# talha-alam/ADAM-Dehaze

Measured on AMD Instinct MI355X. Metric: images/sec CORUN-Complex fwd+bwd 512x1024 bs=8; PSNR vs CPU ref, higher is better.
Workload: dtype f32; 1 GPU; CORUN-Complex (HighIntensityDehazeModel base 96) train-mode fwd + L1 + bwd + Adam; per_gpu_batch=8, global_batch=8, height=512, width=1024, parallelism=dp1

## Files before the change

adam-dehaze_amd/_hip.py:

```python
from __future__ import annotations

import ctypes as C
import os
from typing import Optional

import torch

_LIB_PATH = os.environ.get("ADH_LIB_PATH") or os.path.join(os.path.dirname(os.path.abspath(__file__)), "lib",
                                                           "libadamdehaze_hip.so")
_lib: Optional[C.CDLL] = None

ACT_NONE, ACT_RELU = 0, 1
ACT_RELU6, ACT_HARDSWISH, ACT_HARDSIGMOID = 4, 5, 6

i32, i64, f32, f64, vp = C.c_int32, C.c_int64, C.c_float, C.c_double, C.c_void_p


class ConvDesc(C.Structure):
    _fields_ = [
        ("in_", vp), ("out", vp), ("wp", vp), ("scale", vp), ("shift", vp), ("residual", vp), ("stats", vp),
        ("N", i32), ("IH", i32), ("IW", i32), ("Cin", i32), ("in_cstride", i32),
        ("OH", i32), ("OW", i32), ("Cout", i32), ("out_cstride", i32), ("res_cstride", i32),
        ("VH", i32), ("VW", i32),
        ("in_sy", i32), ("in_sx", i32),
# ... 31 lines not shown
        ("K", i32), ("Nc", i32), ("KHt", i32), ("KWt", i32),
        ("tap_off0", i32), ("tap_off_sy", i32), ("tap_off_sx", i32),
        ("stride_k", i32), ("stride_n", i32),
    ]


PD = C.POINTER(ConvDesc)
PL = C.POINTER(WLayout)

_SIGNATURES = {
    "adh_version": [],
    "adh_conv_lds_bytes": [PD],
    "adh_conv_num_blocks": [PD],
    "adh_pack_weights": [vp, vp, PL, vp],
    "adh_conv_forward": [vp, PD],
    "adh_conv_wino_supported": [PD],
    "adh_conv_wino_forward": [vp, PD],
    "adh_conv_wino_num_blocks": [PD],
    "adh_conv_wino32_supported": [PD],
    "adh_conv_wino32_num_blocks": [PD],
    "adh_conv_wino32_forward": [vp, PD],
    "adh_conv_wino32_forward_multi": [vp, PD, i32],
    "adh_pack_weights_wino32": [vp, vp, PL, vp],
    "adh_conv_wino32_forward_bf16x3": [vp, PD],
    "adh_conv_wino32_forward_multi_bf16x3": [vp, PD, i32],
    "adh_pack_weights_wino32_bf16x3": [vp, vp, PL, vp],
    "adh_conv_wino43_supported": [PD],
    "adh_conv_wino43_num_blocks": [PD],
    "adh_conv_wino43_forward": [vp, PD],
    "adh_conv_wino43_dgrad_bnred": [vp, PD, vp],
    "adh_pack_weights_wino43": [vp, vp, PL, vp],
    "adh_conv_wino43_set_persistent": [i32],
    "adh_conv_wino43_forward_bf16x3": [vp, PD],
    "adh_conv_wino43_dgrad_bnred_bf16x3": [vp, PD, vp],
    "adh_pack_weights_wino43_bf16x3": [vp, vp, PL, vp],
    "adh_pack_weights_wino": [vp, vp, PL, vp],
    "adh_conv_wgrad": [vp, PD, vp, i32],
    "adh_conv_wgrad_wino_groups": [PD],
    "adh_conv_wgrad_wino": [vp, PD, vp, i32],
    "adh_wgrad_reduce_wino": [vp, vp, i32, i32, i32, PL, vp, i32],
    "adh_conv_wgrad_wino32_groups": [PD],
    "adh_conv_wgrad_wino32_classes": [PD],
    "adh_conv_wgrad_wino32_tiles": [PD],
    "adh_conv_wgrad_wino32_launches": [PD],
    "adh_conv_wgrad_wino32": [vp, PD, vp, i32],
    "adh_conv_wgrad_wino32_multi": [vp, PD, i32, vp, i32],
# ... 120 lines not shown
    "adh_bn_slice_stats_num_blocks": [i64, i32],
    "adh_bn_slice_stats": [vp, vp, i32, i64, i32, vp],
    "adh_bn_slice_moments": [vp, vp, i32, i32, i32, f64, vp, vp],
    "adh_bn_fold_moments": [vp, i32, vp, vp, f64, vp, vp, f32, f32, vp, vp, vp, vp, vp, vp, vp],
    "adh_avgpool2_bwd": [vp, vp, i32, i32, i32, i32, i32, vp, i32, i32],
    "adh_bn_preact_bwd_accum": [vp, vp, i32, vp, i32, vp, vp, vp, vp, i32, vp, i32, i64, i32, i32],
    "adh_u8_to_image": [vp, vp, i64, i64, i32, i32, i32, i32, vp],
    "adh_image_to_u8": [vp, vp, i32, i32, i32, vp, i64, i64, i32],
    "adh_ciede2000_num_blocks": [i64],
    "adh_ciede2000": [vp, vp, vp, i32, i32, i32, i32, vp, i32, vp, vp],
    "adh_d4_apply": [vp, vp, i32, i32, i32, i32, i32, i32, vp, vp, i32, f32],
    "adh_msssim_num_tiles": [i32, i32],
    "adh_msssim_level_fwd": [vp, vp, vp, i32, i32, i32, i32, f64, vp, i32, vp, vp, vp, vp],
    "adh_msssim_level_bwd": [vp, vp, vp, i32, i32, i32, i32, f64, vp, vp, vp, vp, i32],
    "adh_draw_boxes": [vp, vp, i64, i64, i32, i32, i32, i32, vp, i32, vp, vp, vp, i32, vp, i32, i32, i32, i32],
    "adh_u8_resize_bilinear": [vp, vp, i64, i32, i32, i32, vp, i32, i32],
    "adh_batch_num_blocks": [i64],
    "adh_batch_from_u8": [vp, vp, i64, i64, i32, i32, vp, vp, i32, vp, i32, vp],
    "adh_batch_window_from_u8": [vp, vp, i64, vp, vp, i32, i32, i32, vp, i32, vp],
    "adh_nss_halve": [vp, vp, i32, i32, i32, i32, i32, i32, vp],
    "adh_nss_moments": [vp, vp, i32, i32, i32, i32, i32, i32, i32, i32, vp, i32, vp],
}

_VALUE_FUNCS = {"adh_version", "adh_conv_fewout_supported", "adh_conv_fewin_supported", "adh_conv_fewin_num_blocks", "adh_conv_wgrad_wino32_launches", "adh_conv_wino_supported", "adh_conv_wino_num_blocks", "adh_conv_wino32_supported", "adh_conv_wino43_supported", "adh_conv_wino43_num_blocks", "adh_conv_wino43_set_persistent",
                "adh_conv_wino32_num_blocks", "adh_conv_wgrad_wino_groups", "adh_conv_wgrad_wino32_groups", "adh_conv_wgrad_wino32_classes", "adh_conv_wgrad_wino32_tiles", "adh_conv_wgrad_wino43_groups", "adh_conv_wgrad_wino43_strips", "adh_conv_wgrad_small_slabs", "adh_conv_wgrad_stem_slabs", "adh_conv_stem_num_blocks", "adh_conv_wgrad_slabs", "adh_conv_wgrad_groups", "adh_conv_lds_bytes", "adh_conv_num_blocks", "adh_bn_bwd_num_blocks",
                "adh_cbam_pool_num_blocks", "adh_cbam_bwd_b_num_blocks", "adh_head_blend_bwd_num_blocks",
                "adh_reduce_num_blocks", "adh_lpips_layer_num_blocks", "adh_adam_chunk_elems", "adh_nms_words", "adh_augment_num_blocks", "adh_psnr_num_blocks", "adh_cbam_bwd_d_scratch_floats",
                "adh_ssim_num_blocks", "adh_fft_l1_workspace_bytes", "adh_fft_l1_num_partials", "adh_dwconv_num_blocks", "adh_dwconv_wgrad_num_blocks", "adh_channel_scale_bwd_num_blocks",
                "adh_bn_slice_stats_num_blocks", "adh_ciede2000_num_blocks", "adh_msssim_num_tiles", "adh_batch_num_blocks"}

_ERRORS = {-1: "ADH_E_ARG (bad argument: shape / alignment / null pointer)",
           -2: "ADH_E_LAUNCH (hip kernel launch failed)",
           -3: "ADH_E_UNSUPPORTED (configuration not supported by the kernels)"}


def lib_path() -> str:
    return _LIB_PATH


def load() -> C.CDLL:
    global _lib
    if _lib is None:
        if not os.path.exists(_LIB_PATH):
            raise RuntimeError(
                f"{_LIB_PATH} not found: the HIP extension is not built (run `python -c 'import __graft_entry__ as g; "
                "g.build()'` or `make -C adam-dehaze_amd/csrc`). There is no CPU fallback on the product path.")
        lib = C.CDLL(_LIB_PATH)
# ... 72 lines not shown
```

adam-dehaze_amd/csrc/conv_wino.hip:

```cpp
#include "common.h"
#ifndef W_STORE_AUX
#define W_STORE_AUX 0
#endif
#ifndef W3_DBG
#define W3_DBG 0
#endif
#include <cstdlib>
#include <cstring>
#define B3_NO_SPLIT ((W3_DBG & 16) != 0)
#include "bf16x3.h"

#define W2_KC 16
#define W2_TILES 64
#define W2_VBUF_F (16 * W2_TILES * W2_KC)
#define W2_RAW_PITCH 576
#define W2_RAW_F (10 * W2_RAW_PITCH)
#define W2_LDS_BYTES ((2 * W2_VBUF_F + W2_RAW_F) * 4)

typedef __attribute__((address_space(3))) void* lds_void_ptr;

struct WinoGeom {
    int tiles_x, tiles_y;
    int nregions;
    int nchunks;
    int KQtot;
    int ncog;
    int dbg;
};

template <int NT, int FT, int J>
constexpr bool w2_in_agpr() {
    constexpr int nv = 8 * NT - 16;
    if constexpr (nv <= 0) return true;
    else return !(J == 0 && FT >= 8 - nv);
}
template <bool AGPR>
__device__ __forceinline__ void w2_mfma(f32x16& c, float a, float b) {
    if constexpr (AGPR) asm("v_mfma_f32_32x32x2_f32 %0, %1, %2, %0" : "+a"(c) : "v"(a), "v"(b));
    else asm("v_mfma_f32_32x32x2_f32 %0, %1, %2, %0" : "+v"(c) : "v"(a), "v"(b));
}
template <int NT, int J, int FT, int R>
__device__ __forceinline__ void w2_store_m(const f32x16 (&acc)[8 * NT], unsigned addr) {
    if constexpr (FT < 8) {
        constexpr int off = ((FT >> 1) * W2_TILES + 8 * (R >> 2) + ((R & 3) << 1) + 32 * (FT & 1)) * 128;
        if constexpr (w2_in_agpr<NT, FT, J>())
            asm volatile("ds_write_b32 %0, %1 offset:%2" ::"v"(addr), "a"(acc[FT * NT + J][R]), "n"(off) : "memory");
        else
            asm volatile("ds_write_b32 %0, %1 offset:%2" ::"v"(addr), "v"(acc[FT * NT + J][R]), "n"(off) : "memory");
        if constexpr (R + 1 < 16) w2_store_m<NT, J, FT, R + 1>(acc, addr);
        else w2_store_m<NT, J, FT + 1, 0>(acc, addr);
    }
}

template <int NT, int F, int KK, int TH, int J, int KEND = 4>
__device__ __forceinline__ void w2_group(f32x16 (&acc)[8 * NT], const f32x4 (&a)[2], const f32x4 (&b)[NT]) {
    if constexpr (KK < KEND) {
        w2_mfma<w2_in_agpr<NT, F * 2 + TH, J>()>(acc[(F * 2 + TH) * NT + J], a[TH][KK], b[J][KK]);
        if constexpr (J + 1 < NT) w2_group<NT, F, KK, TH, J + 1, KEND>(acc, a, b);
        else if constexpr (TH == 0) w2_group<NT, F, KK, 1, 0, KEND>(acc, a, b);
        else w2_group<NT, F, KK + 1, 0, 0, KEND>(acc, a, b);
    }
}

template <int NT>
__device__ __forceinline__ void w2_load_b(f32x4 (&b)[NT], unsigned voff, const float* sbase) {
    asm volatile("global_load_dwordx4 %0, %1, %2" : "=v"(b[0]) : "v"(voff), "s"(sbase) : "memory");
    if constexpr (NT > 1) asm volatile("global_load_dwordx4 %0, %1, %2 offset:512" : "=v"(b[1]) : "v"(voff), "s"(sbase) : "memory");
    if constexpr (NT > 2) asm volatile("global_load_dwordx4 %0, %1, %2 offset:1024" : "=v"(b[2]) : "v"(voff), "s"(sbase) : "memory");
}
template <int N, int NT>
__device__ __forceinline__ void w2_wait_b(f32x4 (&b)[NT]) {
    if constexpr (NT == 1) asm volatile("s_waitcnt vmcnt(%1)" : "+v"(b[0]) : "n"(N) : "memory");
    if constexpr (NT == 2) asm volatile("s_waitcnt vmcnt(%2)" : "+v"(b[0]), "+v"(b[1]) : "n"(N) : "memory");
    if constexpr (NT == 3) asm volatile("s_waitcnt vmcnt(%3)" : "+v"(b[0]), "+v"(b[1]), "+v"(b[2]) : "n"(N) : "memory");
}

template <int NT>
__global__ __launch_bounds__(256, 1) void conv_wino_kernel(const adh_conv_desc d, const WinoGeom g) {
    extern __shared__ __attribute__((aligned(16))) float lds[];
    float* const raw = lds + 2 * W2_VBUF_F;

    const int tid = threadIdx.x;
    const int lane = tid & 63;
// ... 496 lines not shown
            }
            asm volatile("s_nop 1" : "+v"(a[0][0]), "+v"(a[0][1]), "+v"(a[0][2]), "+v"(a[1][0]), "+v"(a[1][1]), "+v"(a[1][2]));
        } else {
            w3b_gap<NT, FI, 12 * J + 12>(n, v0, v1, m1);
        }
        w3b_groups<NT, G + 1>(acc, a, n, bv, v0, v1, b_voff, b_slab, m1, st, sgn, nbuf);
    }
}

struct Wino32Geom {
    int tiles_x, tiles_y;
    int nregions;
    int nchunks;
    int KQtot;
    int ncog;
    int ncls, xps;
    int ymin[4], xmin[4];
    int wcls;
    int nmerge, mblocks;
    int region0;
    int m_out_oy[4], m_out_ox[4];
    const float* m_wp[4];
    float* m_stats[4];
};

template <int NT, bool BF3 = false>
__global__ __launch_bounds__(256, 1) void conv_wino32_kernel(const adh_conv_desc d, const Wino32Geom g) {
    extern __shared__ __attribute__((aligned(16))) float lds[];
    float* const rawbase = lds + W2_VBUF_F;
    float* const red = rawbase + 2 * W3_RAW_F;

    const int tid = threadIdx.x;
    const int lane = tid & 63;
    const int wave = __builtin_amdgcn_readfirstlane(tid >> 6);
    const int l31 = lane & 31;
    const int h = lane >> 5;

    const int bid = (int)blockIdx.x;
    const int gq = bid >> 3, per_region = g.ncog * g.nmerge;
    const int r8 = gq / per_region, rem = gq - r8 * per_region;
    const int mc = rem / g.ncog;
    const float* const wp_m = g.nmerge > 1 ? g.m_wp[mc] : d.wp;
    float* const stats_m = g.nmerge > 1 ? g.m_stats[mc] : d.stats;
    const int out_oy_m = g.nmerge > 1 ? g.m_out_oy[mc] : d.out_oy, out_ox_m = g.nmerge > 1 ? g.m_out_ox[mc] : d.out_ox;
    W3_STAMP(0);
#ifdef W3_PROF
    if (tid == 0 && bid < 16384) {
        w3_prof_buf[bid * 32 + 6] = __builtin_amdgcn_s_getreg((4 << 0) | (0 << 6) | (31 << 11));
        w3_prof_buf[bid * 32 + 7] = __builtin_amdgcn_s_getreg((20 << 0) | (0 << 6) | (31 << 11));
    }
#endif
    const int cg = rem - mc * g.ncog;
    const int region = g.region0 + r8 * 8 + (bid & 7);
    if (region >= g.nregions) return;
    int rr = region;
    const int tx = rr % g.tiles_x;
    rr /= g.tiles_x;
    const int ty = rr % g.tiles_y;
    const int n = rr / g.tiles_y;
    const int vy0 = ty * 12, vx0 = tx * 48;
    const int co0 = cg * 32 * NT;

    const int xcs = d.in_cstride * 4 * g.xps;
    const int xrs = d.IW * d.in_cstride * 4 * g.xps;
    const float* const in_n = d.in + (int64_t)n * d.IH * d.IW * d.in_cstride;
    const __amdgpu_buffer_rsrc_t xr = __builtin_amdgcn_make_buffer_rsrc(const_cast<float*>(in_n), 0, 0x7fffffff, 0x00020000);
    const int cq_l = lane & 3, px_l = lane >> 2;
    const int vfull = 3 * px_l * xcs + cq_l * 16;
    const int vtail = (px_l < W3_RAW_ROWS ? px_l : 0) * xrs + 48 * xcs + cq_l * 16;
    typedef W3Slab SlabGeom;
    auto slab_geom = [&](int slab) {
        SlabGeom sg;
        const int chunk = slab / g.ncls, c = slab - chunk * g.ncls;
        sg.iy0 = vy0 * g.xps + g.ymin[c + mc];
        sg.ix0 = vx0 * g.xps + g.xmin[c + mc];
        sg.interior = sg.iy0 >= 0 && sg.iy0 + 12 * g.xps < d.IH && sg.ix0 >= 0 && sg.ix0 + 48 * g.xps < d.IW;
// ... 15 lines not shown
                    __builtin_amdgcn_raw_ptr_buffer_load_lds(xr, (lds_void_ptr)(raw + r * W3_RAW_PITCH + p * 256), 16, vfull,
                                                             __builtin_amdgcn_readfirstlane(so0 + r * xrs + p * xcs), 0, 0);
                } else {
                    __builtin_amdgcn_raw_ptr_buffer_load_lds(xr, (lds_void_ptr)(raw + W3_RAW_ROWS * W3_RAW_PITCH), 16, vtail,
                                                             __builtin_amdgcn_readfirstlane(so0), 0, 0);
                }
            }
        } else {
#pragma unroll
            for (int u = u0; u < u1; ++u) {
                const int j = 4 * u + wv;
                const bool tail = j >= 39;
                const int rs = (j * 171) >> 9, p = tail ? 0 : j - rs * 3;
                const int r = tail ? (px_l < W3_RAW_ROWS ? px_l : 0) : rs;
                const int col = tail ? 48 : 3 * px_l + p;
                const int iy = iy0 + r * g.xps, ix = ix0 + col * g.xps;
                const bool ok = iy >= 0 && iy < d.IH && ix >= 0 && ix < d.IW;
                const int vo = ok ? (iy * d.IW + ix) * d.in_cstride * 4 + cq_l * 16 : (int)0x80000000;
                const int doff = __builtin_amdgcn_readfirstlane(tail ? W3_RAW_ROWS * W3_RAW_PITCH : rs * W3_RAW_PITCH + p * 256);
                __builtin_amdgcn_raw_ptr_buffer_load_lds(xr, (lds_void_ptr)(raw + doff), 16, vo, __builtin_amdgcn_readfirstlane(cb), 0, 0);
            }
        }
    };
    const int tcol = lane >> 2;
    const int tile_t = wave * 16 + tcol;
    int colb[3], colb3[4];
#pragma unroll
    for (int b = 0; b < 3; ++b) colb[b] = (3 * wave) * W3_RAW_PITCH + b * 256 + tcol * 16 + cq_l * 4;
#pragma unroll
    for (int i = 0; i < 4; ++i)
        colb3[i] = (tcol < 15 ? (3 * wave + i) * W3_RAW_PITCH + (tcol + 1) * 16 : W3_RAW_ROWS * W3_RAW_PITCH + (3 * wave + i) * 16) + cq_l * 4;
    const int vslot_t = tile_t * 16 + ((cq_l ^ ((tile_t >> 1) & 3)) * 4);
    const float m1 = adh_opaque(-1.f);
    auto transform = [&](int buf) {
        const float* raw = rawbase + buf * W3_RAW_F;
        float* Vb = lds + vslot_t;
#pragma unroll
        for (int a = 0; a < 4; ++a) {
            const int rA = a == 0 ? 0 : (a == 2 ? 2 : 1), rB = a == 0 ? 2 : (a == 1 ? 2 : (a == 2 ? 1 : 3));
            f32x4 t[4];
#pragma unroll
            for (int b = 0; b < 4; ++b) {
                const f32x4 dA = *reinterpret_cast<const f32x4*>(b < 3 ? raw + colb[b] + rA * W3_RAW_PITCH : raw + colb3[rA]);
                const f32x4 dB = *reinterpret_cast<const f32x4*>(b < 3 ? raw + colb[b] + rB * W3_RAW_PITCH : raw + colb3[rB]);
                t[b] = a == 1 ? dA + dB : adh_pksub(dA, dB, m1);
            }
            *reinterpret_cast<f32x4*>(Vb + (a * 4 + 0) * 1024) = adh_pksub(t[0], t[2], m1);
            *reinterpret_cast<f32x4*>(Vb + (a * 4 + 1) * 1024) = t[1] + t[2];
            *reinterpret_cast<f32x4*>(Vb + (a * 4 + 2) * 1024) = adh_pksub(t[2], t[1], m1);
            *reinterpret_cast<f32x4*>(Vb + (a * 4 + 3) * 1024) = adh_pksub(t[1], t[3], m1);
        }
    };

    const int sw = (l31 >> 1) & 3;
// ... 6 lines not shown
    f32x16 acc[8 * NT];
#pragma unroll
    for (int t = 0; t < 8 * NT; ++t)
#pragma unroll
        for (int r = 0; r < 16; ++r) acc[t][r] = 0.f;

    const float* const v0 = lds + a_lane;
    const float* const v1 = lds + (a_lane ^ 8);
    const unsigned b3_voff = (unsigned)lane * 16u;
    const size_t b3_chunk = (size_t)16 * NT * 3072, b3_cls = (size_t)g.ncog * g.nchunks * b3_chunk;
    const char* const b3_wave = reinterpret_cast<const char*>(wp_m) + ((size_t)cg * g.nchunks * 16 + (size_t)wave * 4) * (NT * 3072);
    auto b3_ptr = [&](int slab) {
        const int chunk = slab / g.ncls, c = slab - chunk * g.ncls;
        return b3_wave + (size_t)c * b3_cls + (size_t)chunk * b3_chunk;
    };
    W3Stage st3;
    st3.xr = xr; st3.rawbase = rawbase; st3.vfull = vfull; st3.vtail = vtail; st3.wave = wave; st3.px_l = px_l; st3.cq_l = cq_l;
    st3.xps = g.xps; st3.IH = d.IH; st3.IW = d.IW; st3.in_cstride = d.in_cstride; st3.xcs = xcs; st3.xrs = xrs;
    u32x4 av3[2][3], bv3[3][3];
    W4BNext nx[2];
    const float m1s = adh_opaque(-1.f);

    f32x4 av[2][2], bv[2][NT];
    auto load_a = [&](int f, int gg, f32x4 (&a)[2]) {
        const float* p = lds + f * 1024 + (gg ? (a_lane ^ 8) : a_lane);
        a[0] = *reinterpret_cast<const f32x4*>(p);
        a[1] = *reinterpret_cast<const f32x4*>(p + 512);
    };
    auto b_ptr = [&](int slab, int f, int gg) {
        const int chunk = slab / g.ncls, c = slab - chunk * g.ncls;
        return b_wave + (int64_t)c * g.wcls + f * b_fstride + (int64_t)(chunk * 4 + 2 * gg) * b_kqstride;
    };

    const int nslabs = g.nchunks * g.ncls;
    if constexpr (!BF3) w2_load_b<NT>(bv[0], b_voff, b_ptr(0, 0, 0));
    stage_raw(slab_geom(0), 0, 0, 10);
    asm volatile("s_waitcnt vmcnt(0)" ::: "memory");
    __builtin_amdgcn_s_barrier();
    if (!(W3_DBG & 1)) transform(0);
    asm volatile("s_waitcnt lgkmcnt(0)" ::: "memory");
    __builtin_amdgcn_s_barrier();

    W3_STAMP(1);
#pragma unroll 1
    for (int s = 0; s < nslabs; ++s) {
        if (s == 1) W3_STAMP(8);
        const int sn = s + 1 < nslabs ? s + 1 : s;
        constexpr int P = (W3_DBG & 8) ? 0 : 2;
        const SlabGeom sgn = slab_geom(sn);
        if constexpr (BF3) {
            if (!(W3_DBG & 2)) {
                w4b_load_b(bv3[0], b3_voff, b3_ptr(s));
                w4b_load_b(bv3[1], b3_voff, b3_ptr(s) + 3072);
                w3b_load_s(nx, v0, v1);
                w3b_steps<0, 40>(nx, m1s);
#pragma unroll
                for (int th = 0; th < 2; ++th) {
                    av3[th][0] = u32x4{nx[th].h[0], nx[th].h[1], nx[th].h[2], nx[th].h[3]};
                    av3[th][1] = u32x4{nx[th].m[0], nx[th].m[1], nx[th].m[2], nx[th].m[3]};
                    av3[th][2] = u32x4{nx[th].l[0], nx[th].l[1], nx[th].l[2], nx[th].l[3]};
                }
                asm volatile("s_nop 1" : "+v"(av3[0][0]), "+v"(av3[0][1]), "+v"(av3[0][2]), "+v"(av3[1][0]), "+v"(av3[1][1]), "+v"(av3[1][2]));
                w3b_load_s(nx, v0 + 1024, v1 + 1024);
                __builtin_amdgcn_sched_barrier(0);
                w3b_groups<NT, 0>(acc, av3, nx, bv3, v0, v1, b3_voff, b3_ptr(s), m1s, st3, sgn, (s + 1) & 1);
                asm volatile("s_waitcnt vmcnt(0)" ::: "memory");
            }
        } else if (!(W3_DBG & 2)) {
        load_a(0, 0, av[0]);
        w2_load_b<NT>(bv[1], b_voff, b_ptr(s, 1, 0));
        load_a(1, 0, av[1]);
        w2_wait_b<NT, NT>(bv[0]);
        w2_group<NT, 0, 0, 0, 0>(acc, av[0], bv[0]);

#define W3_GROUP_WITH_PIECES(F_, CUR, U0)                                             \
        w2_group<NT, F_, 0, 0, 0, 1>(acc, av[CUR], bv[CUR]);                           \
        __builtin_amdgcn_sched_barrier(0);                                            \
        if (P) stage_raw(sgn, (s + 1) & 1, U0, U0 + 2);                               \
        __builtin_amdgcn_sched_barrier(0);                                            \
        w2_group<NT, F_, 1, 0, 0>(acc, av[CUR], bv[CUR]);

        w2_load_b<NT>(bv[0], b_voff, b_ptr(s, 2, 0));
        load_a(2, 0, av[0]);
        w2_wait_b<NT, NT>(bv[1]);
        W3_GROUP_WITH_PIECES(1, 1, 0)

        w2_load_b<NT>(bv[1], b_voff, b_ptr(s, 3, 0));
        load_a(3, 0, av[1]);
        w2_wait_b<NT + P, NT>(bv[0]);
        W3_GROUP_WITH_PIECES(2, 0, 2)

        w2_load_b<NT>(bv[0], b_voff, b_ptr(s, 0, 1));
        load_a(0, 1, av[0]);
        w2_wait_b<NT + P, NT>(bv[1]);
        W3_GROUP_WITH_PIECES(3, 1, 4)

        w2_load_b<NT>(bv[1], b_voff, b_ptr(s, 1, 1));
        load_a(1, 1, av[1]);
        w2_wait_b<NT + P, NT>(bv[0]);
        W3_GROUP_WITH_PIECES(0, 0, 6)

        w2_load_b<NT>(bv[0], b_voff, b_ptr(s, 2, 1));
        load_a(2, 1, av[0]);
        w2_wait_b<NT + P, NT>(bv[1]);
        W3_GROUP_WITH_PIECES(1, 1, 8)
#undef W3_GROUP_WITH_PIECES

        w2_load_b<NT>(bv[1], b_voff, b_ptr(s, 3, 1));
        load_a(3, 1, av[1]);
        w2_wait_b<NT + P, NT>(bv[0]);
        w2_group<NT, 2, 0, 0, 0>(acc, av[0], bv[0]);

        w2_load_b<NT>(bv[0], b_voff, b_ptr(sn, 0, 0));
        w2_wait_b<NT, NT>(bv[1]);
        w2_group<NT, 3, 0, 0, 0>(acc, av[1], bv[1]);
        }
        if (s == 1) W3_STAMP(9);
        asm volatile("s_waitcnt lgkmcnt(0)" ::: "memory");
        __builtin_amdgcn_s_barrier();
        if (s == 1) W3_STAMP(10);
        if (!(W3_DBG & 1)) transform((s + 1) & 1);
        asm volatile("s_waitcnt lgkmcnt(0)" ::: "memory");
        if (s == 1) W3_STAMP(11);
        __builtin_amdgcn_s_barrier();
        if (s == 1) W3_STAMP(12);
    }
    if constexpr (!BF3) w2_wait_b<0, NT>(bv[0]);
    W3_STAMP(2);

    if (W3_DBG & 4) return;
    float* M = lds;
    const int eq = tid & 7;
    float* out_n = d.out + (size_t)n * d.OH * d.OW * d.out_cstride;
    const float* res_n = d.residual ? d.residual + (size_t)n * d.OH * d.OW * d.res_cstride : nullptr;
    const int o_px = d.out_cstride * 4 * d.out_sx, o_row = d.OW * d.out_cstride * 4 * d.out_sy;
    const int r_px = d.res_cstride * 4 * d.out_sx, r_row = d.OW * d.res_cstride * 4 * d.out_sy;
    const __amdgpu_buffer_rsrc_t orsrc = __builtin_amdgcn_make_buffer_rsrc(out_n, 0, 0x7fffffff, 0x00020000);
    const __amdgpu_buffer_rsrc_t rrsrc =
        __builtin_amdgcn_make_buffer_rsrc(const_cast<float*>(res_n ? res_n : out_n), 0, 0x7fffffff, 0x00020000);
    const bool ragged = vy0 + 12 > d.VH || vx0 + 48 > d.VW;
    const float act_lo = d.act == ADH_ACT_RELU ? 0.f : -INFINITY;
    const unsigned m_wbase = (unsigned)(((wave * 4) * W2_TILES + h) * 32 + l31) * 4u;
    typedef unsigned u32x4 __attribute__((ext_vector_type(4)));
#pragma unroll
    for (int j = 0; j < NT; ++j) {
        if (j == 1) W3_STAMP(16);
        __builtin_amdgcn_s_barrier();
        if (j == 1) W3_STAMP(17);
        if (j == 0) w2_store_m<NT, 0, 0, 0>(acc, m_wbase);
        if (j == 1) w2_store_m<NT, (NT > 1 ? 1 : 0), 0, 0>(acc, m_wbase);
        if (j == 2) w2_store_m<NT, (NT > 2 ? 2 : 0), 0, 0>(acc, m_wbase);
        asm volatile("s_waitcnt lgkmcnt(0)" ::: "memory");
        if (j == 1) W3_STAMP(18);
        __builtin_amdgcn_s_barrier();
        if (j == 1) W3_STAMP(19);
        const int cq0 = co0 + j * 32 + eq * 4;
        const bool quad_ok = cq0 + 3 < d.Cout;
        f32x4 sc4 = {1.f, 1.f, 1.f, 1.f}, sh4 = {0.f, 0.f, 0.f, 0.f};
        if (d.scale && quad_ok) sc4 = *reinterpret_cast<const f32x4*>(d.scale + cq0);
        if (d.shift && quad_ok) sh4 = *reinterpret_cast<const f32x4*>(d.shift + cq0);
        const unsigned chanpen = quad_ok ? 0u : 0x80000000u;
        f32x4 ssum = {0.f, 0.f, 0.f, 0.f}, ssq = {0.f, 0.f, 0.f, 0.f};
#pragma unroll
        for (int p = 0; p < 2; ++p) {
            const int t = (tid >> 3) + 32 * p;
            const int tp = (t & ~7) | ((t & 3) << 1) | ((t >> 2) & 1);
            const float* mp = M + tp * 32 + eq * 4;
            const int vyb = vy0 + 3 * (t >> 4), vxb = vx0 + 3 * (t & 15);
            unsigned rowpen[3], colpen[3];
            float rowf[3], colf[3];
#pragma unroll
            for (int r = 0; r < 3; ++r) {
                rowpen[r] = vyb + r < d.VH ? 0u : 0x80000000u;
                colpen[r] = vxb + r < d.VW ? 0u : 0x80000000u;
                rowf[r] = vyb + r < d.VH ? 1.f : 0.f;
                colf[r] = vxb + r < d.VW ? 1.f : 0.f;
            }
            const int pix0 = (vyb * d.out_sy + out_oy_m) * d.OW + vxb * d.out_sx + out_ox_m;
            const unsigned o_vj = (unsigned)(pix0 * d.out_cstride * 4 + cq0 * 4) | chanpen;
            const unsigned r_vj = (unsigned)(pix0 * d.res_cstride * 4 + cq0 * 4) | chanpen;
            f32x4 rres[9];
            if (res_n) {
#pragma unroll
                for (int i = 0; i < 3; ++i)
#pragma unroll
                    for (int jj = 0; jj < 3; ++jj)
                        rres[i * 3 + jj] = __builtin_bit_cast(
                            f32x4, __builtin_amdgcn_raw_buffer_load_b128(rrsrc, r_vj | rowpen[i] | colpen[jj], i * r_row + jj * r_px, 0));
                asm volatile("" ::: "memory");
            } else {
#pragma unroll
// ... 42 lines not shown
                for (int o = 8; o < 64; o <<= 1) {
                    ssum[e] += __shfl_xor(ssum[e], o, 64);
                    ssq[e] += __shfl_xor(ssq[e], o, 64);
                }
            }
            if (j) __builtin_amdgcn_s_barrier();
            if (lane < 8) {
                *reinterpret_cast<f32x4*>(red + (0 * 4 + wave) * 32 + eq * 4) = ssum;
                *reinterpret_cast<f32x4*>(red + (1 * 4 + wave) * 32 + eq * 4) = ssq;
            }
            asm volatile("s_waitcnt lgkmcnt(0)" ::: "memory");
            __builtin_amdgcn_s_barrier();
            if (tid < 64) {
                const int which = tid >> 5, cl = tid & 31;
                float v = 0.f;
#pragma unroll
                for (int r = 0; r < 4; ++r) v += red[(which * 4 + r) * 32 + cl];
                stats_m[((size_t)region * 2 + which) * d.NcP + co0 + j * 32 + cl] = v;
            }
        }
    }
    W3_STAMP(3);
}

static int wino32_plan(const adh_conv_desc* d, Wino32Geom* g) {
    static const bool enabled = !(getenv("ADH_WINO32") && atoi(getenv("ADH_WINO32")) == 0);
    if (!enabled || !d) return 0;
    if (d->Cin % W2_KC != 0 || d->in_cstride % 4 != 0 || d->NcP % 32 != 0) return 0;
    if (d->in_sy != d->in_sx || d->dstep_y != d->dstep_x || d->out_sy != d->out_sx) return 0;
    if ((int64_t)(d->IH + 2) * d->IW * d->in_cstride >= (1ll << 29)) return 0;
    if (d->Cout % 4 != 0 || d->out_cstride % 4 != 0 || ((uintptr_t)d->out & 15) || (int64_t)d->OH * d->OW * d->out_cstride >= (1ll << 29))
        return 0;
    if (d->residual && (d->res_cstride % 4 != 0 || ((uintptr_t)d->residual & 15) ||
                        (int64_t)d->OH * d->OW * d->res_cstride >= (1ll << 29)))
        return 0;
    if ((d->scale && ((uintptr_t)d->scale & 15)) || (d->shift && ((uintptr_t)d->shift & 15))) return 0;
    if (d->KH == 2 && d->KW == 2 && d->dstep_y == d->in_sy && (d->in_sy == 1 || d->in_sy == 2)) {
        g->ncls = 1; g->xps = d->in_sy;
        for (int c = 0; c < 4; ++c) { g->ymin[c] = d->dy0; g->xmin[c] = d->dx0; }
    } else if (d->KH == 4 && d->KW == 4 && d->in_sy == 2 && d->dstep_y == 1) {
        g->ncls = 4; g->xps = 2;
        for (int py = 0; py < 2; ++py)
            for (int px = 0; px < 2; ++px) { g->ymin[py * 2 + px] = d->dy0 + py; g->xmin[py * 2 + px] = d->dx0 + px; }
    } else {
        return 0;
    }
    g->tiles_x = adh_ceil_div(d->VW, 48);
    g->tiles_y = adh_ceil_div(d->VH, 12);
    g->nregions = g->tiles_x * g->tiles_y * d->N;
    g->nchunks = d->Cin / W2_KC;
    g->KQtot = d->Cin / 4;
    g->wcls = 16 * g->KQtot * d->NcP * 4;
    g->nmerge = 1;
    g->region0 = 0;
    g->mblocks = 0;
    return 1;
}

extern "C" int adh_conv_wino32_supported(const adh_conv_desc* d) {
    Wino32Geom g;
    return wino32_plan(d, &g);
}

extern "C" int adh_conv_wino32_num_blocks(const adh_conv_desc* d) {
    Wino32Geom g;
    if (!wino32_plan(d, &g)) return ADH_E_UNSUPPORTED;
    return g.nregions;
}

static int wino32_tail_split(int nregions, int group_blocks , int NT) {
    static int ncu = -1;
    if (ncu < 0) {
        int dev = 0;
        hipDeviceProp_t p;
        ncu = (hipGetDevice(&dev) == hipSuccess && hipGetDeviceProperties(&p, dev) == hipSuccess) ? p.multiProcessorCount : 256;
        const char* e = getenv("ADH_WINO32_TAIL");
        if (e && atoi(e) == 0) ncu = 0;
    }
// ... 21 lines not shown
    return adh_check_launch();
}
template <int NT, bool BF3 = false>
static int launch_wino32(hipStream_t s, const adh_conv_desc* d, Wino32Geom g) {
    const int nreg = g.nregions;
    const int main_regions = BF3 ? nreg : wino32_tail_split(nreg, 8 * (d->NcP / (32 * NT)), NT);
    const int rc = launch_wino32_part<NT, BF3>(s, d, g, 0, main_regions);
    if (rc || main_regions == nreg) return rc;
    return launch_wino32_part<1, BF3>(s, d, g, main_regions, nreg);
}

static int wino32_forward_impl(void* stream, const adh_conv_desc* d, bool bf3) {
    Wino32Geom g;
    if (!wino32_plan(d, &g)) return ADH_E_UNSUPPORTED;
    if (!d->in || !d->out || !d->wp || d->NcP < d->Cout) return ADH_E_ARG;
    if (d->out_cstride < d->Cout || (d->residual && d->res_cstride < d->Cout)) return ADH_E_ARG;
    if ((d->VH - 1) * d->out_sy + d->out_oy >= d->OH || (d->VW - 1) * d->out_sx + d->out_ox >= d->OW || d->out_oy < 0 ||
        d->out_ox < 0)
        return ADH_E_ARG;
    if (((uintptr_t)d->in & 15) || ((uintptr_t)d->wp & 15)) return ADH_E_ARG;
    const int nt = d->NcP / 32;
    hipStream_t s = (hipStream_t)stream;
    if (bf3) {
        if (nt % 3 == 0) return launch_wino32<3, true>(s, d, g);
        if (nt % 2 == 0) return launch_wino32<2, true>(s, d, g);
        return launch_wino32<1, true>(s, d, g);
    }
    if (nt % 3 == 0) return launch_wino32<3>(s, d, g);
    if (nt % 2 == 0) return launch_wino32<2>(s, d, g);
    return launch_wino32<1>(s, d, g);
}

extern "C" int adh_conv_wino32_forward(void* stream, const adh_conv_desc* d) { return wino32_forward_impl(stream, d, false); }
extern "C" int adh_conv_wino32_forward_bf16x3(void* stream, const adh_conv_desc* d) { return wino32_forward_impl(stream, d, true); }

static int wino32_forward_multi_impl(void* stream, const adh_conv_desc* descs, int n, bool bf3) {
    if (!descs || n < 1 || n > 4) return ADH_E_ARG;
    if (n == 1) return wino32_forward_impl(stream, descs, bf3);
    Wino32Geom g0;
    if (!wino32_plan(&descs[0], &g0) || g0.ncls != 1) return ADH_E_UNSUPPORTED;
    for (int m = 0; m < n; ++m) {
        const adh_conv_desc* d = &descs[m];
        Wino32Geom g;
        if (!wino32_plan(d, &g) || g.ncls != 1) return ADH_E_UNSUPPORTED;
        if (!d->in || !d->out || !d->wp || d->NcP < d->Cout) return ADH_E_ARG;
        if (d->out_cstride < d->Cout || (d->residual && d->res_cstride < d->Cout)) return ADH_E_ARG;
        if ((d->VH - 1) * d->out_sy + d->out_oy >= d->OH || (d->VW - 1) * d->out_sx + d->out_ox >= d->OW || d->out_oy < 0 ||
            d->out_ox < 0)
            return ADH_E_ARG;
        if (((uintptr_t)d->in & 15) || ((uintptr_t)d->wp & 15)) return ADH_E_ARG;
        adh_conv_desc a = descs[0], b = *d;
        a.wp = b.wp = nullptr; a.stats = b.stats = nullptr;
        a.out_oy = b.out_oy = 0; a.out_ox = b.out_ox = 0; a.dy0 = b.dy0 = 0; a.dx0 = b.dx0 = 0;
        if (memcmp(&a, &b, sizeof(a)) != 0 || (!descs[0].stats) != (!d->stats)) return ADH_E_UNSUPPORTED;
        g0.ymin[m] = g.ymin[0]; g0.xmin[m] = g.xmin[0];
        g0.m_out_oy[m] = d->out_oy; g0.m_out_ox[m] = d->out_ox;
        g0.m_wp[m] = d->wp; g0.m_stats[m] = d->stats;
    }
    for (int m = n; m < 4; ++m) {
        g0.ymin[m] = g0.ymin[0]; g0.xmin[m] = g0.xmin[0];
        g0.m_out_oy[m] = 0; g0.m_out_ox[m] = 0; g0.m_wp[m] = nullptr; g0.m_stats[m] = nullptr;
    }
    const int nt = descs[0].NcP / 32;
    const int NT = nt % 3 == 0 ? 3 : (nt % 2 == 0 ? 2 : 1);
    hipStream_t s = (hipStream_t)stream;
    const int nreg = g0.nregions;
    const int main_regions = bf3 ? nreg : wino32_tail_split(nreg, 8 * n * (descs[0].NcP / (32 * NT)), NT);
    for (int part = 0; part < 2; ++part) {
        const int r0 = part ? main_regions : 0, r1 = part ? nreg : main_regions, nt_part = part ? 1 : NT;
        if (r1 <= r0) break;
        g0.ncog = descs[0].NcP / (32 * nt_part);
        g0.nmerge = n;
        g0.region0 = r0;
        g0.nregions = r1;
        g0.mblocks = ((r1 - r0 + 7) / 8) * g0.ncog * 8;
        const int nblocks = n * g0.mblocks;
#define W3_LAUNCH_MULTI(NT_, BF_)                                                                                                       \
        do {                                                                                                                             \
            (void)hipFuncSetAttribute(reinterpret_cast<const void*>(&conv_wino32_kernel<NT_, BF_>), hipFuncAttributeMaxDynamicSharedMemorySize, \
                                      160 * 1024);                                                                                       \
            hipLaunchKernelGGL((conv_wino32_kernel<NT_, BF_>), dim3(nblocks), dim3(256), W3_LDS_BYTES, s, descs[0], g0);                 \
        } while (0)
        if (bf3) {
            if (nt_part == 3) W3_LAUNCH_MULTI(3, true);
            else if (nt_part == 2) W3_LAUNCH_MULTI(2, true);
// ... 207 lines not shown
```

include/adam_dehaze_hip.h:

```cpp
#ifndef ADAM_DEHAZE_HIP_H
#define ADAM_DEHAZE_HIP_H

#include <stdint.h>

#ifdef __cplusplus
extern "C" {
#endif

#define ADH_OK 0
#define ADH_E_ARG (-1)
#define ADH_E_LAUNCH (-2)
#define ADH_E_UNSUPPORTED (-3)

#define ADH_ACT_NONE 0
#define ADH_ACT_RELU 1
#define ADH_ACT_SIGMOID 2
#define ADH_ACT_TANH 3
#define ADH_ACT_RELU6 4
#define ADH_ACT_HARDSWISH 5
#define ADH_ACT_HARDSIGMOID 6

typedef struct adh_conv_desc {
    const float* in;
    float* out;
// ... 16 lines not shown
typedef struct adh_wlayout {
    int32_t K, Nc;
    int32_t KHt, KWt;
    int32_t tap_off0, tap_off_sy, tap_off_sx;
    int32_t stride_k, stride_n;
} adh_wlayout;

int adh_version(void);
int adh_conv_lds_bytes(const adh_conv_desc* d);
int adh_conv_num_blocks(const adh_conv_desc* d);

int adh_pack_weights(void* stream, const float* src, const adh_wlayout* L, float* wp);

int adh_conv_forward(void* stream, const adh_conv_desc* d);
int adh_conv_wino_supported(const adh_conv_desc* d);
int adh_conv_wino_forward(void* stream, const adh_conv_desc* d);
int adh_conv_wino_num_blocks(const adh_conv_desc* d);
int adh_pack_weights_wino(void* stream, const float* src, const adh_wlayout* L, float* wp);
int adh_conv_wino32_supported(const adh_conv_desc* d);
int adh_conv_wino32_num_blocks(const adh_conv_desc* d);
int adh_conv_wino32_forward(void* stream, const adh_conv_desc* d);
int adh_conv_wino32_forward_multi(void* stream, const adh_conv_desc* descs, int n);
int adh_pack_weights_wino32(void* stream, const float* src, const adh_wlayout* L, float* wp);
int adh_conv_wino32_forward_bf16x3(void* stream, const adh_conv_desc* d);
int adh_conv_wino32_forward_multi_bf16x3(void* stream, const adh_conv_desc* descs, int n);
int adh_pack_weights_wino32_bf16x3(void* stream, const float* src, const adh_wlayout* L, void* wp);

int adh_conv_wino43_supported(const adh_conv_desc* d);
int adh_conv_wino43_num_blocks(const adh_conv_desc* d);
int adh_conv_wino43_forward(void* stream, const adh_conv_desc* d);
int adh_conv_wino43_dgrad_bnred(void* stream, const adh_conv_desc* d, const float* bn_mean);
int adh_pack_weights_wino43(void* stream, const float* src, const adh_wlayout* L, float* wp);
int adh_conv_wino43_set_persistent(int on);
int adh_conv_wino43_forward_bf16x3(void* stream, const adh_conv_desc* d);
int adh_conv_wino43_dgrad_bnred_bf16x3(void* stream, const adh_conv_desc* d, const float* bn_mean);
int adh_pack_weights_wino43_bf16x3(void* stream, const float* src, const adh_wlayout* L, void* wp);

int adh_conv_wgrad_small_slabs(const adh_conv_desc* d);
int adh_conv_wgrad_small(void* stream, const adh_conv_desc* d, float* slab, int KP, int NcP);
int adh_wgrad_reduce_small(void* stream, const float* slab, int nslabs, int KP, int NcP, const adh_wlayout* L, float* dst,
                           int accumulate);

int adh_conv_fewout_supported(const adh_conv_desc* d);
int adh_conv_fewout_forward(void* stream, const adh_conv_desc* d);
int adh_pack_weights_fewout(void* stream, const float* src, const adh_wlayout* L, float* wp);
int adh_conv_fewin_supported(const adh_conv_desc* d);
// ... 303 lines not shown
```

Before: 40.45 images/sec.

## Skip dead half-tiles at image edges in Winograd F(2,3) conv kernel

Adds an edge-skip mode to the wino32 forward kernel. When the second half of a block's tile region lies outside the valid output, only half the MFMA groups, A loads, transforms, M stores and epilogue passes run. A tile layout (rows vs column halves) is chosen per shape to minimise live work, and a region rotation (xrot) is added to spread edge blocks across the block index. The mode is on by default via an env flag. It adds code duplication from two instantiated slab loops, which raises code size and possibly register pressure, and the bf16x3 path keeps it disabled.

```diff
diff --git a/adam-dehaze_amd/_hip.py b/adam-dehaze_amd/_hip.py
--- a/adam-dehaze_amd/_hip.py
+++ b/adam-dehaze_amd/_hip.py
@@ -77,6 +77,8 @@
     "adh_conv_wino32_forward": [vp, PD],
     "adh_conv_wino32_forward_multi": [vp, PD, i32],
     "adh_pack_weights_wino32": [vp, vp, PL, vp],
+    "adh_w32_set_edge_skip": [i32],
+    "adh_w32_live_blocks": [i32, i32, i32],
     "adh_conv_wino32_forward_bf16x3": [vp, PD],
     "adh_conv_wino32_forward_multi_bf16x3": [vp, PD, i32],
     "adh_pack_weights_wino32_bf16x3": [vp, vp, PL, vp],
@@ -243,7 +245,7 @@
     "adh_nss_moments": [vp, vp, i32, i32, i32, i32, i32, i32, i32, i32, vp, i32, vp],
 }
 
-_VALUE_FUNCS = {"adh_version", "adh_conv_fewout_supported", "adh_conv_fewin_supported", "adh_conv_fewin_num_blocks", "adh_conv_wgrad_wino32_launches", "adh_conv_wino_supported", "adh_conv_wino_num_blocks", "adh_conv_wino32_supported", "adh_conv_wino43_supported", "adh_conv_wino43_num_blocks", "adh_conv_wino43_set_persistent",
+_VALUE_FUNCS = {"adh_version", "adh_conv_fewout_supported", "adh_conv_fewin_supported", "adh_conv_fewin_num_blocks", "adh_conv_wgrad_wino32_launches", "adh_conv_wino_supported", "adh_conv_wino_num_blocks", "adh_conv_wino32_supported", "adh_conv_wino43_supported", "adh_conv_wino43_num_blocks", "adh_conv_wino43_set_persistent", "adh_w32_set_edge_skip", "adh_w32_live_blocks",
                 "adh_conv_wino32_num_blocks", "adh_conv_wgrad_wino_groups", "adh_conv_wgrad_wino32_groups", "adh_conv_wgrad_wino32_classes", "adh_conv_wgrad_wino32_tiles", "adh_conv_wgrad_wino43_groups", "adh_conv_wgrad_wino43_strips", "adh_conv_wgrad_small_slabs", "adh_conv_wgrad_stem_slabs", "adh_conv_stem_num_blocks", "adh_conv_wgrad_slabs", "adh_conv_wgrad_groups", "adh_conv_lds_bytes", "adh_conv_num_blocks", "adh_bn_bwd_num_blocks",
                 "adh_cbam_pool_num_blocks", "adh_cbam_bwd_b_num_blocks", "adh_head_blend_bwd_num_blocks",
                 "adh_reduce_num_blocks", "adh_lpips_layer_num_blocks", "adh_adam_chunk_elems", "adh_nms_words", "adh_augment_num_blocks", "adh_psnr_num_blocks", "adh_cbam_bwd_d_scratch_floats",
diff --git a/adam-dehaze_amd/csrc/conv_wino.hip b/adam-dehaze_amd/csrc/conv_wino.hip
--- a/adam-dehaze_amd/csrc/conv_wino.hip
+++ b/adam-dehaze_amd/csrc/conv_wino.hip
@@ -39,26 +39,28 @@
     if constexpr (AGPR) asm("v_mfma_f32_32x32x2_f32 %0, %1, %2, %0" : "+a"(c) : "v"(a), "v"(b));
     else asm("v_mfma_f32_32x32x2_f32 %0, %1, %2, %0" : "+v"(c) : "v"(a), "v"(b));
 }
-template <int NT, int J, int FT, int R>
+template <int NT, int J, int FT, int R, int NB = 2>
 __device__ __forceinline__ void w2_store_m(const f32x16 (&acc)[8 * NT], unsigned addr) {
-    if constexpr (FT < 8) {
+    if constexpr (FT < 8 && NB == 1 && (FT & 1)) {
+        w2_store_m<NT, J, FT + 1, 0, NB>(acc, addr);
+    } else if constexpr (FT < 8) {
         constexpr int off = ((FT >> 1) * W2_TILES + 8 * (R >> 2) + ((R & 3) << 1) + 32 * (FT & 1)) * 128;
         if constexpr (w2_in_agpr<NT, FT, J>())
             asm volatile("ds_write_b32 %0, %1 offset:%2" ::"v"(addr), "a"(acc[FT * NT + J][R]), "n"(off) : "memory");
         else
             asm volatile("ds_write_b32 %0, %1 offset:%2" ::"v"(addr), "v"(acc[FT * NT + J][R]), "n"(off) : "memory");
-        if constexpr (R + 1 < 16) w2_store_m<NT, J, FT, R + 1>(acc, addr);
-        else w2_store_m<NT, J, FT + 1, 0>(acc, addr);
-    }
-}
-
-template <int NT, int F, int KK, int TH, int J, int KEND = 4>
+        if constexpr (R + 1 < 16) w2_store_m<NT, J, FT, R + 1, NB>(acc, addr);
+        else w2_store_m<NT, J, FT + 1, 0, NB>(acc, addr);
+    }
+}
+
+template <int NT, int F, int KK, int TH, int J, int KEND = 4, int NB = 2>
 __device__ __forceinline__ void w2_group(f32x16 (&acc)[8 * NT], const f32x4 (&a)[2], const f32x4 (&b)[NT]) {
     if constexpr (KK < KEND) {
         w2_mfma<w2_in_agpr<NT, F * 2 + TH, J>()>(acc[(F * 2 + TH) * NT + J], a[TH][KK], b[J][KK]);
-        if constexpr (J + 1 < NT) w2_group<NT, F, KK, TH, J + 1, KEND>(acc, a, b);
-        else if constexpr (TH == 0) w2_group<NT, F, KK, 1, 0, KEND>(acc, a, b);
-        else w2_group<NT, F, KK + 1, 0, 0, KEND>(acc, a, b);
+        if constexpr (J + 1 < NT) w2_group<NT, F, KK, TH, J + 1, KEND, NB>(acc, a, b);
+        else if constexpr (TH == 0 && NB == 2) w2_group<NT, F, KK, 1, 0, KEND, NB>(acc, a, b);
+        else w2_group<NT, F, KK + 1, 0, 0, KEND, NB>(acc, a, b);
     }
 }
 
@@ -601,6 +603,8 @@
     int m_out_oy[4], m_out_ox[4];
     const float* m_wp[4];
     float* m_stats[4];
+    int layout, edge_skip;
+    int xrot;
 };
 
 template <int NT, bool BF3 = false>
@@ -630,7 +634,7 @@
     }
 #endif
     const int cg = rem - mc * g.ncog;
-    const int region = g.region0 + r8 * 8 + (bid & 7);
+    const int region = g.region0 + r8 * 8 + ((bid + g.xrot * r8) & 7);
     if (region >= g.nregions) return;
     int rr = region;
     const int tx = rr % g.tiles_x;
@@ -692,14 +696,18 @@
             }
         }
     };
-    const int tcol = lane >> 2;
-    const int tile_t = wave * 16 + tcol;
+    const int tslot = lane >> 2;
+    const int tile_t = wave * 16 + tslot;
+    const int trow = g.layout ? (wave & 1) * 2 + (tslot >> 3) : wave;
+    const int tcol = g.layout ? (wave >> 1) * 8 + (tslot & 7) : tslot;
+    const bool live1 = BF3 || !g.edge_skip || (g.layout ? vx0 + 24 < d.VW : vy0 + 6 < d.VH);
+    const bool tlive = live1 || wave < 2;
     int colb[3], colb3[4];
 #pragma unroll
-    for (int b = 0; b < 3; ++b) colb[b] = (3 * wave) * W3_RAW_PITCH + b * 256 + tcol * 16 + cq_l * 4;
+    for (int b = 0; b < 3; ++b) colb[b] = (3 * trow) * W3_RAW_PITCH + b * 256 + tcol * 16 + cq_l * 4;
 #pragma unroll
     for (int i = 0; i < 4; ++i)
-        colb3[i] = (tcol < 15 ? (3 * wave + i) * W3_RAW_PITCH + (tcol + 1) * 16 : W3_RAW_ROWS * W3_RAW_PITCH + (3 * wave + i) * 16) + cq_l * 4;
+        colb3[i] = (tcol < 15 ? (3 * trow + i) * W3_RAW_PITCH + (tcol + 1) * 16 : W3_RAW_ROWS * W3_RAW_PITCH + (3 * trow + i) * 16) + cq_l * 4;
     const int vslot_t = tile_t * 16 + ((cq_l ^ ((tile_t >> 1) & 3)) * 4);
     const float m1 = adh_opaque(-1.f);
     auto transform = [&](int buf) {
@@ -752,10 +760,10 @@
     const float m1s = adh_opaque(-1.f);
 
     f32x4 av[2][2], bv[2][NT];
-    auto load_a = [&](int f, int gg, f32x4 (&a)[2]) {
+    auto load_a = [&](int f, int gg, f32x4 (&a)[2], bool both) {
         const float* p = lds + f * 1024 + (gg ? (a_lane ^ 8) : a_lane);
         a[0] = *reinterpret_cast<const f32x4*>(p);
-        a[1] = *reinterpret_cast<const f32x4*>(p + 512);
+        if (both) a[1] = *reinterpret_cast<const f32x4*>(p + 512);
     };
     auto b_ptr = [&](int slab, int f, int gg) {
         const int chunk = slab / g.ncls, c = slab - chunk * g.ncls;
@@ -767,95 +775,102 @@
     stage_raw(slab_geom(0), 0, 0, 10);
     asm volatile("s_waitcnt vmcnt(0)" ::: "memory");
     __builtin_amdgcn_s_barrier();
-    if (!(W3_DBG & 1)) transform(0);
+    if (!(W3_DBG & 1) && tlive) transform(0);
     asm volatile("s_waitcnt lgkmcnt(0)" ::: "memory");
     __builtin_amdgcn_s_barrier();
 
     W3_STAMP(1);
-#pragma unroll 1
-    for (int s = 0; s < nslabs; ++s) {
-        if (s == 1) W3_STAMP(8);
-        const int sn = s + 1 < nslabs ? s + 1 : s;
-        constexpr int P = (W3_DBG & 8) ? 0 : 2;
-        const SlabGeom sgn = slab_geom(sn);
-        if constexpr (BF3) {
-            if (!(W3_DBG & 2)) {
-                w4b_load_b(bv3[0], b3_voff, b3_ptr(s));
-                w4b_load_b(bv3[1], b3_voff, b3_ptr(s) + 3072);
-                w3b_load_s(nx, v0, v1);
-                w3b_steps<0, 40>(nx, m1s);
-#pragma unroll
-                for (int th = 0; th < 2; ++th) {
-                    av3[th][0] = u32x4{nx[th].h[0], nx[th].h[1], nx[th].h[2], nx[th].h[3]};
-                    av3[th][1] = u32x4{nx[th].m[0], nx[th].m[1], nx[th].m[2], nx[th].m[3]};
-                    av3[th][2] = u32x4{nx[th].l[0], nx[th].l[1], nx[th].l[2], nx[th].l[3]};
-                }
-                asm volatile("s_nop 1" : "+v"(av3[0][0]), "+v"(av3[0][1]), "+v"(av3[0][2]), "+v"(av3[1][0]), "+v"(av3[1][1]), "+v"(av3[1][2]));
-                w3b_load_s(nx, v0 + 1024, v1 + 1024);
-                __builtin_amdgcn_sched_barrier(0);
-                w3b_groups<NT, 0>(acc, av3, nx, bv3, v0, v1, b3_voff, b3_ptr(s), m1s, st3, sgn, (s + 1) & 1);
-                asm volatile("s_waitcnt vmcnt(0)" ::: "memory");
-            }
-        } else if (!(W3_DBG & 2)) {
-        load_a(0, 0, av[0]);
-        w2_load_b<NT>(bv[1], b_voff, b_ptr(s, 1, 0));
-        load_a(1, 0, av[1]);
-        w2_wait_b<NT, NT>(bv[0]);
-        w2_group<NT, 0, 0, 0, 0>(acc, av[0], bv[0]);
-
-#define W3_GROUP_WITH_PIECES(F_, CUR, U0)                                             \
-        w2_group<NT, F_, 0, 0, 0, 1>(acc, av[CUR], bv[CUR]);                           \
+#define W3_GROUP_WITH_PIECES(NB, F_, CUR, U0)                                         \
+        w2_group<NT, F_, 0, 0, 0, 1, NB>(acc, av[CUR], bv[CUR]);                       \
         __builtin_amdgcn_sched_barrier(0);                                            \
         if (P) stage_raw(sgn, (s + 1) & 1, U0, U0 + 2);                               \
         __builtin_amdgcn_sched_barrier(0);                                            \
-        w2_group<NT, F_, 1, 0, 0>(acc, av[CUR], bv[CUR]);
-
-        w2_load_b<NT>(bv[0], b_voff, b_ptr(s, 2, 0));
-        load_a(2, 0, av[0]);
-        w2_wait_b<NT, NT>(bv[1]);
-        W3_GROUP_WITH_PIECES(1, 1, 0)
-
-        w2_load_b<NT>(bv[1], b_voff, b_ptr(s, 3, 0));
-        load_a(3, 0, av[1]);
-        w2_wait_b<NT + P, NT>(bv[0]);
-        W3_GROUP_WITH_PIECES(2, 0, 2)
-
-        w2_load_b<NT>(bv[0], b_voff, b_ptr(s, 0, 1));
-        load_a(0, 1, av[0]);
-        w2_wait_b<NT + P, NT>(bv[1]);
-        W3_GROUP_WITH_PIECES(3, 1, 4)
-
-        w2_load_b<NT>(bv[1], b_voff, b_ptr(s, 1, 1));
-        load_a(1, 1, av[1]);
-        w2_wait_b<NT + P, NT>(bv[0]);
-        W3_GROUP_WITH_PIECES(0, 0, 6)
-
-        w2_load_b<NT>(bv[0], b_voff, b_ptr(s, 2, 1));
-        load_a(2, 1, av[0]);
-        w2_wait_b<NT + P, NT>(bv[1]);
-        W3_GROUP_WITH_PIECES(1, 1, 8)
+        w2_group<NT, F_, 1, 0, 0, 4, NB>(acc, av[CUR], bv[CUR]);
+#define W3_SLAB_LOOP(NB)                                                              \
+    _Pragma("unroll 1")                                                               \
+    for (int s = 0; s < nslabs; ++s) {                                                \
+        if (s == 1) W3_STAMP(8);                                                      \
+        const int sn = s + 1 < nslabs ? s + 1 : s;                                    \
+        constexpr int P = (W3_DBG & 8) ? 0 : 2;                                       \
+        const SlabGeom sgn = slab_geom(sn);                                           \
+        if constexpr (BF3) {                                                          \
+            if (!(W3_DBG & 2)) {                                                      \
+                w4b_load_b(bv3[0], b3_voff, b3_ptr(s));                               \
+                w4b_load_b(bv3[1], b3_voff, b3_ptr(s) + 3072);                        \
+                w3b_load_s(nx, v0, v1);                                               \
+                w3b_steps<0, 40>(nx, m1s);                                            \
+                _Pragma("unroll")                                                     \
+                for (int th = 0; th < 2; ++th) {                                      \
+                    av3[th][0] = u32x4{nx[th].h[0], nx[th].h[1], nx[th].h[2], nx[th].h[3]}; \
+                    av3[th][1] = u32x4{nx[th].m[0], nx[th].m[1], nx[th].m[2], nx[th].m[3]}; \
+                    av3[th][2] = u32x4{nx[th].l[0], nx[th].l[1], nx[th].l[2], nx[th].l[3]}; \
+                }                                                                     \
+                asm volatile("s_nop 1" : "+v"(av3[0][0]), "+v"(av3[0][1]), "+v"(av3[0][2]), "+v"(av3[1][0]), "+v"(av3[1][1]), "+v"(av3[1][2])); \
+                w3b_load_s(nx, v0 + 1024, v1 + 1024);                                 \
+                __builtin_amdgcn_sched_barrier(0);                                    \
+                w3b_groups<NT, 0>(acc, av3, nx, bv3, v0, v1, b3_voff, b3_ptr(s), m1s, st3, sgn, (s + 1) & 1); \
+                asm volatile("s_waitcnt vmcnt(0)" ::: "memory");                      \
+            }                                                                         \
+        } else if (!(W3_DBG & 2)) {                                                   \
+        load_a(0, 0, av[0], NB == 2);                                                 \
+        w2_load_b<NT>(bv[1], b_voff, b_ptr(s, 1, 0));                                 \
+        load_a(1, 0, av[1], NB == 2);                                                 \
+        w2_wait_b<NT, NT>(bv[0]);                                                     \
+        w2_group<NT, 0, 0, 0, 0, 4, NB>(acc, av[0], bv[0]);                            \
+                                                                                      \
+        w2_load_b<NT>(bv[0], b_voff, b_ptr(s, 2, 0));                                 \
+        load_a(2, 0, av[0], NB == 2);                                                 \
+        w2_wait_b<NT, NT>(bv[1]);                                                     \
+        W3_GROUP_WITH_PIECES(NB, 1, 1, 0)                                             \
+                                                                                      \
+        w2_load_b<NT>(bv[1], b_voff, b_ptr(s, 3, 0));                                 \
+        load_a(3, 0, av[1], NB == 2);                                                 \
+        w2_wait_b<NT + P, NT>(bv[0]);                                                 \
+        W3_GROUP_WITH_PIECES(NB, 2, 0, 2)                                             \
+                                                                                      \
+        w2_load_b<NT>(bv[0], b_voff, b_ptr(s, 0, 1));                                 \
+        load_a(0, 1, av[0], NB == 2);                                                 \
+        w2_wait_b<NT + P, NT>(bv[1]);                                                 \
+        W3_GROUP_WITH_PIECES(NB, 3, 1, 4)                                             \
+                                                                                      \
+        w2_load_b<NT>(bv[1], b_voff, b_ptr(s, 1, 1));                                 \
+        load_a(1, 1, av[1], NB == 2);                                                 \
+        w2_wait_b<NT + P, NT>(bv[0]);                                                 \
+        W3_GROUP_WITH_PIECES(NB, 0, 0, 6)                                             \
+                                                                                      \
+        w2_load_b<NT>(bv[0], b_voff, b_ptr(s, 2, 1));                                 \
+        load_a(2, 1, av[0], NB == 2);                                                 \
+        w2_wait_b<NT + P, NT>(bv[1]);                                                 \
+        W3_GROUP_WITH_PIECES(NB, 1, 1, 8)                                             \
+                                                                                      \
+        w2_load_b<NT>(bv[1], b_voff, b_ptr(s, 3, 1));                                 \
+        load_a(3, 1, av[1], NB == 2);                                                 \
+        w2_wait_b<NT + P, NT>(bv[0]);                                                 \
+        w2_group<NT, 2, 0, 0, 0, 4, NB>(acc, av[0], bv[0]);                            \
+                                                                                      \
+        w2_load_b<NT>(bv[0], b_voff, b_ptr(sn, 0, 0));                                \
+        w2_wait_b<NT, NT>(bv[1]);    \
+        w2_group<NT, 3, 0, 0, 0, 4, NB>(acc, av[1], bv[1]);                            \
+        }                                                                             \
+         \
+        if (s == 1) W3_STAMP(9);                                                      \
+        asm volatile("s_waitcnt lgkmcnt(0)" ::: "memory");                            \
+        __builtin_amdgcn_s_barrier();                                                 \
+        if (s == 1) W3_STAMP(10);                                                     \
+        if (!(W3_DBG & 1) && (NB == 2 || wave < 2)) transform((s + 1) & 1);           \
+        asm volatile("s_waitcnt lgkmcnt(0)" ::: "memory");                            \
+        if (s == 1) W3_STAMP(11);                                                     \
+        __builtin_amdgcn_s_barrier();                                                 \
+        if (s == 1) W3_STAMP(12);                                                     \
+    }                                                                                 \
+    if constexpr (!BF3) w2_wait_b<0, NT>(bv[0]);
+    if (live1) {
+        W3_SLAB_LOOP(2)
+    } else {
+        W3_SLAB_LOOP(1)
+    }
+#undef W3_SLAB_LOOP
 #undef W3_GROUP_WITH_PIECES
-
-        w2_load_b<NT>(bv[1], b_voff, b_ptr(s, 3, 1));
-        load_a(3, 1, av[1]);
-        w2_wait_b<NT + P, NT>(bv[0]);
-        w2_group<NT, 2, 0, 0, 0>(acc, av[0], bv[0]);
-
-        w2_load_b<NT>(bv[0], b_voff, b_ptr(sn, 0, 0));
-        w2_wait_b<NT, NT>(bv[1]);
-        w2_group<NT, 3, 0, 0, 0>(acc, av[1], bv[1]);
-        }
-        if (s == 1) W3_STAMP(9);
-        asm volatile("s_waitcnt lgkmcnt(0)" ::: "memory");
-        __builtin_amdgcn_s_barrier();
-        if (s == 1) W3_STAMP(10);
-        if (!(W3_DBG & 1)) transform((s + 1) & 1);
-        asm volatile("s_waitcnt lgkmcnt(0)" ::: "memory");
-        if (s == 1) W3_STAMP(11);
-        __builtin_amdgcn_s_barrier();
-        if (s == 1) W3_STAMP(12);
-    }
-    if constexpr (!BF3) w2_wait_b<0, NT>(bv[0]);
     W3_STAMP(2);
 
     if (W3_DBG & 4) return;
@@ -877,9 +892,15 @@
         if (j == 1) W3_STAMP(16);
         __builtin_amdgcn_s_barrier();
         if (j == 1) W3_STAMP(17);
-        if (j == 0) w2_store_m<NT, 0, 0, 0>(acc, m_wbase);
-        if (j == 1) w2_store_m<NT, (NT > 1 ? 1 : 0), 0, 0>(acc, m_wbase);
-        if (j == 2) w2_store_m<NT, (NT > 2 ? 2 : 0), 0, 0>(acc, m_wbase);
+        if (live1) {
+            if (j == 0) w2_store_m<NT, 0, 0, 0>(acc, m_wbase);
+            if (j == 1) w2_store_m<NT, (NT > 1 ? 1 : 0), 0, 0>(acc, m_wbase);
+            if (j == 2) w2_store_m<NT, (NT > 2 ? 2 : 0), 0, 0>(acc, m_wbase);
+        } else {
+            if (j == 0) w2_store_m<NT, 0, 0, 0, 1>(acc, m_wbase);
+            if (j == 1) w2_store_m<NT, (NT > 1 ? 1 : 0), 0, 0, 1>(acc, m_wbase);
+            if (j == 2) w2_store_m<NT, (NT > 2 ? 2 : 0), 0, 0, 1>(acc, m_wbase);
+        }
         asm volatile("s_waitcnt lgkmcnt(0)" ::: "memory");
         if (j == 1) W3_STAMP(18);
         __builtin_amdgcn_s_barrier();
@@ -893,10 +914,12 @@
         f32x4 ssum = {0.f, 0.f, 0.f, 0.f}, ssq = {0.f, 0.f, 0.f, 0.f};
 #pragma unroll
         for (int p = 0; p < 2; ++p) {
+            if (p == 1 && !live1) break;
             const int t = (tid >> 3) + 32 * p;
             const int tp = (t & ~7) | ((t & 3) << 1) | ((t >> 2) & 1);
             const float* mp = M + tp * 32 + eq * 4;
-            const int vyb = vy0 + 3 * (t >> 4), vxb = vx0 + 3 * (t & 15);
+            const int trow_e = g.layout ? (t >> 3) & 3 : t >> 4, tcol_e = g.layout ? 8 * p + (t & 7) : t & 15;
+            const int vyb = vy0 + 3 * trow_e, vxb = vx0 + 3 * tcol_e;
             unsigned rowpen[3], colpen[3];
             float rowf[3], colf[3];
 #pragma unroll
@@ -985,6 +1008,29 @@
     }
     W3_STAMP(3);
 }
+
+static int w32_edge_skip = -1;
+static int w32_edge_skip_on() {
+    if (w32_edge_skip < 0) {
+        const char* e = getenv("ADH_W32_EDGE_SKIP");
+        w32_edge_skip = (e && atoi(e) == 0) ? 0 : 1;
+    }
+    return w32_edge_skip;
+}
+extern "C" int adh_w32_set_edge_skip(int on) {
+    const int old = w32_edge_skip_on();
+    w32_edge_skip = on ? 1 : 0;
+    return old;
+}
+extern "C" int adh_w32_live_blocks(int VH, int VW, int layout) {
+    if (VH < 1 || VW < 1 || layout < 0 || layout > 1) return ADH_E_ARG;
+    const int ry = adh_ceil_div(VH, 12), rx = adh_ceil_div(VW, 48);
+    int live = ry * rx;
+    if (layout == 0) live += rx * ((VH - 6 + 11) / 12);
+    else live += ry * ((VW - 24 + 47) / 48);
+    return live;
+}
+static int w32_pick_layout(int VH, int VW) { return adh_w32_live_blocks(VH, VW, 1) < adh_w32_live_blocks(VH, VW, 0) ? 1 : 0; }
 
 static int wino32_plan(const adh_conv_desc* d, Wino32Geom* g) {
     static const bool enabled = !(getenv("ADH_WINO32") && atoi(getenv("ADH_WINO32")) == 0);
@@ -1017,6 +1063,9 @@
     g->nmerge = 1;
     g->region0 = 0;
     g->mblocks = 0;
+    g->edge_skip = w32_edge_skip_on();
+    g->layout = g->edge_skip ? w32_pick_layout(d->VH, d->VW) : 0;
+    g->xrot = g->layout == 1 && g->tiles_x % 2 == 0;
     return 1;
 }
 
@@ -1084,6 +1133,7 @@
     const int nt = d->NcP / 32;
     hipStream_t s = (hipStream_t)stream;
     if (bf3) {
+        g.layout = g.edge_skip = g.xrot = 0;
         if (nt % 3 == 0) return launch_wino32<3, true>(s, d, g);
         if (nt % 2 == 0) return launch_wino32<2, true>(s, d, g);
         return launch_wino32<1, true>(s, d, g);
@@ -1123,6 +1173,7 @@
         g0.ymin[m] = g0.ymin[0]; g0.xmin[m] = g0.xmin[0];
         g0.m_out_oy[m] = 0; g0.m_out_ox[m] = 0; g0.m_wp[m] = nullptr; g0.m_stats[m] = nullptr;
     }
+    if (bf3) g0.layout = g0.edge_skip = g0.xrot = 0;
     const int nt = descs[0].NcP / 32;
     const int NT = nt % 3 == 0 ? 3 : (nt % 2 == 0 ? 2 : 1);
     hipStream_t s = (hipStream_t)stream;
diff --git a/include/adam_dehaze_hip.h b/include/adam_dehaze_hip.h
--- a/include/adam_dehaze_hip.h
+++ b/include/adam_dehaze_hip.h
@@ -62,6 +62,8 @@
 int adh_conv_wino32_forward(void* stream, const adh_conv_desc* d);
 int adh_conv_wino32_forward_multi(void* stream, const adh_conv_desc* descs, int n);
 int adh_pack_weights_wino32(void* stream, const float* src, const adh_wlayout* L, float* wp);
+int adh_w32_set_edge_skip(int on);
+int adh_w32_live_blocks(int VH, int VW, int layout);
 int adh_conv_wino32_forward_bf16x3(void* stream, const adh_conv_desc* d);
 int adh_conv_wino32_forward_multi_bf16x3(void* stream, const adh_conv_desc* descs, int n);
 int adh_pack_weights_wino32_bf16x3(void* stream, const float* src, const adh_wlayout* L, void* wp);
```

Result: no change. 40.43 images/sec (-0.1%).
